# Fro116/RecommenderSystem

Hardware: AMD Instinct MI355X
Metric: interactions/sec (higher is better)
Workload: dtype bf16

## Files before the change

### include/rsys_debug.h

```cpp
#ifndef RSYS_DEBUG_H
#define RSYS_DEBUG_H
#include "rsys.h"

#ifdef __cplusplus
extern "C" {
#endif

int32_t rsys_debug_get(rsys_model* m, const char* key, void* out, int64_t bytes);

int32_t rsys_local_group_create(int32_t world, int32_t device, void** group);
int32_t rsys_local_group_destroy(void* group);
int32_t rsys_comm_init_local(void* group, int32_t rank, rsys_comm** out);
int32_t rsys_comm_debug_delay(rsys_comm* c, int32_t microseconds);

int32_t rsys_dev_alloc(void** p, size_t bytes);
int32_t rsys_dev_free(void* p);
int32_t rsys_dev_h2d(void* dst, const void* src, size_t bytes);
int32_t rsys_dev_d2h(void* dst, const void* src, size_t bytes);
int32_t rsys_dev_memset(void* dst, int value, size_t bytes);
int32_t rsys_op_gemm(int32_t dtype, const void* A, const void* B, void* C, int32_t M, int32_t N, int32_t K,
                     int64_t lda, int64_t ldb, int64_t ldc, int32_t a_km, int32_t b_km, int32_t a_f32, int32_t c_f32,
                     int32_t splitk);
int32_t rsys_op_gemm_rows(int32_t dtype, const void* A, const void* B, void* C, int32_t M, int32_t N, int32_t K,
                          int64_t lda, int64_t ldb, int64_t ldc, int32_t b_km, int32_t c_f32, const int32_t* rows_dev);
// ... 2 lines not shown
int32_t rsys_op_gemm_epi(int32_t dtype, const void* A, const void* B, void* C, int32_t M, int32_t N, int32_t K, int64_t lda,
                         int64_t ldb, int64_t ldc, int32_t b_km, int32_t c_f32, int32_t epi, float alpha, int32_t accum,
                         const float* bias, const float* resid, int64_t ldr, void* C2, int64_t ldc2, const float* E,
                         const float* rope_cos, const float* rope_sin, const float* rope_cs, const int32_t* rope_pos, int32_t T,
                         int32_t hd, int32_t n_q, int32_t n_k, const int32_t* m_dev, char* tag, int32_t tag_bytes, int32_t* half);
int32_t rsys_debug_gemm_route(int32_t dtype, int32_t M, int32_t N, int32_t K, int64_t lda, int64_t ldb, int64_t ldc, int32_t a_km,
                              int32_t b_km, int32_t a_f32, int32_t c_f32, int32_t epi, int32_t splitk, int32_t flags, float alpha,
                              int32_t accum, int32_t set, int32_t m_expect, int32_t cus, char* tag, int32_t tag_bytes, int32_t* splits);
int32_t rsys_op_attention(int32_t dtype, int32_t B, int32_t T, int32_t H, int32_t KV, int32_t hd, const void* qkv,
                          const int32_t* uid, const int32_t* tm, void* O, float* lse, const void* dO, void* dqkv,
                          const float* rope_cos, const float* rope_sin);
int32_t rsys_op_attention_ex(int32_t dtype, int32_t B, int32_t T, int32_t H, int32_t KV, int32_t hd, const void* qkv,
                             const int32_t* uid, const int32_t* tm, void* O, float* lse, const void* dO, void* dqkv,
                             const float* rope_cos, const float* rope_sin, const int32_t* rope_pos, int32_t rope_rows,
                             const int32_t* q_active, float* amax_fwd, float* amax_bwd);
int32_t rsys_op_attention_selected(int32_t dtype, int32_t B, int32_t T, int32_t H, int32_t KV, int32_t hd, const void* qkv,
                                   const int32_t* uid, const int32_t* tm, int32_t n_sel, const int32_t* sel, void* O);
int32_t rsys_op_attention_maps(int32_t dtype, int32_t B, int32_t T, int32_t H, int32_t KV, int32_t hd, const int32_t* uid, const int32_t* tm,
                               const int32_t* q_active, const int32_t* uid_prev, const int32_t* tm_prev, void* qmap, void* kmap,
                               void* qmap_full, void* kmap_full, void* qmap16, void* kmap16, uint64_t* qbits, uint64_t* kbits,
                               int32_t* order_q, int32_t* order_k, int32_t* info);
int32_t rsys_op_attention_cached(int32_t dtype, int32_t rows, int32_t T, int32_t H, int32_t KV, int32_t hd, const void* qkv, const void* cache,
                                 int32_t n_slots, const int32_t* slot, const int32_t* n_hist, const int32_t* n_cand, void* O);
int32_t rsys_op_attention_cached_tiles(int32_t dtype, int32_t rows, int32_t T, int32_t H, int32_t KV, int32_t hd, const void* qkv, const void* cache,
                                       int32_t n_slots, int32_t Tc, int32_t n_seg, const int32_t* seg, void* O);
int32_t rsys_op_rank_cache_copy_segments(int32_t dtype, int32_t rows, int32_t T, int32_t H, int32_t KV, int32_t hd, const void* qkv, void* cache,
                                         int32_t n_slots, int32_t Tc, int32_t n_seg, const int32_t* seg);
int32_t rsys_rank_cache_get(rsys_model* m, int32_t layer, int32_t slot, void* out, int64_t bytes);
int32_t rsys_op_topk(const float* scores, int64_t ld, int32_t rows, int32_t V, int32_t k,
                     int32_t* ids, float* vals, int32_t* counts);
int32_t rsys_op_topk_window(const float* scores, int64_t ld, int32_t rows, int32_t V, const int64_t* start, const int32_t* len,
                            int32_t* ids, float* vals, int32_t* counts, int32_t* totals, int32_t* bounds);
int32_t rsys_op_lse(const float* z, int64_t ldz, int32_t rows, int32_t V, float* lse);
int32_t rsys_op_text_rows(void* search, const float* x, int32_t n, float* z_out, float* lse_out);
int32_t rsys_op_query_weights(const float* z, int64_t ldz, const float* lse, const int32_t* members, const int32_t* ranges, int32_t q0,
                              const float* user_w, int32_t n_groups, const float* src, float* dst, int32_t V, int32_t last,
// ... 100 lines not shown
```

### recommendersystem_amd/_lib.py

```python
import ctypes as C
import os

os.environ.setdefault("HSA_ENABLE_IPC_MODE_LEGACY", "0")

HERE = os.path.dirname(os.path.abspath(__file__))
LIB_PATH = os.path.join(HERE, "librsys_hip.so")


class RsysError(RuntimeError):
    pass


class rsys_config(C.Structure):
    _fields_ = [
        ("num_layers", C.c_int32), ("num_heads", C.c_int32), ("num_kv_heads", C.c_int32),
        ("embed_dim", C.c_int32), ("intermediate_dim", C.c_int32), ("max_sequence_length", C.c_int32),
        ("vocab_0", C.c_int32), ("vocab_1", C.c_int32),
        ("vocab_status", C.c_int32), ("vocab_gender", C.c_int32), ("vocab_source", C.c_int32),
        ("metadata_dim", C.c_int32),
        ("min_ts", C.c_double), ("max_ts", C.c_double),
        ("rating_mean", C.c_float), ("rating_std", C.c_float), ("mask_rate", C.c_float),
        ("mask_topk", C.c_int32), ("finetune", C.c_int32), ("finetune_metric", C.c_int32),
        ("dtype", C.c_int32), ("max_rows", C.c_int32), ("lora_dropout", C.c_float),
        ("table_shard_rank", C.c_int32), ("table_shard_world", C.c_int32), ("sampled_negatives", C.c_int32),
# ... 127 lines not shown
    ("rsys_adapter_forward_backward", C.c_int32, [_P, C.c_int32, _P, _P, C.c_float, C.c_uint64, C.c_uint64]),
    ("rsys_adapter_forward_backward_packed", C.c_int32, [_P, C.c_int32, _P, C.c_int32, C.c_float, C.c_uint64, C.c_uint64]),
    ("rsys_adapter_grad_get", C.c_int32, [_P, C.c_int32, C.c_char_p, _P, C.c_int64]),
    ("rsys_adapter_zero_grad", C.c_int32, [_P]),
    ("rsys_adapter_adamw_step", C.c_int32, [_P, C.c_float, C.c_float, C.c_float, C.c_float, C.c_float, _P, C.c_int32, _P]),
    ("rsys_adapter_adamw_state_get", C.c_int32, [_P, C.c_int32, C.c_char_p, _P, _P, C.c_int64, C.POINTER(C.c_int32)]),
    ("rsys_adapter_adamw_state_set", C.c_int32, [_P, C.c_int32, C.c_char_p, _P, _P, C.c_int64, C.c_int32]),
    ("rsys_rank_cache_reserve", C.c_int32, [_P, C.c_int32]),
    ("rsys_rank_cache_store", C.c_int32, [_P, _P, _P, _P]),
    ("rsys_rank_cache_candidates", C.c_int32, [_P, _P, _P, _P, _P]),
    ("rsys_rank_cache_store_packed", C.c_int32, [_P, _P, C.c_int32, _P]),
    ("rsys_rank_cache_candidates_packed", C.c_int32, [_P, _P, C.c_int32, _P, _P]),
    ("rsys_rank_cache_get", C.c_int32, [_P, C.c_int32, C.c_int32, _P, C.c_int64]),
    ("rsys_op_attention_selected", C.c_int32, [C.c_int32] * 6 + [_P, _P, _P, C.c_int32, _P, _P]),
    ("rsys_op_attention_maps", C.c_int32, [C.c_int32] * 6 + [_P] * 16),
    ("rsys_op_attention_cached", C.c_int32, [C.c_int32] * 6 + [_P, _P, C.c_int32, _P, _P, _P, _P]),
    ("rsys_op_attention_cached_tiles", C.c_int32, [C.c_int32] * 6 + [_P, _P, C.c_int32, C.c_int32, C.c_int32, _P, _P]),
    ("rsys_op_rank_cache_copy_segments", C.c_int32, [C.c_int32] * 6 + [_P, _P, C.c_int32, C.c_int32, C.c_int32, _P]),
    ("rsys_trunk_output_get", C.c_int32, [_P, _P, C.c_int64]),
    ("rsys_debug_get", C.c_int32, [_P, C.c_char_p, _P, C.c_int64]),
    ("rsys_clip_grad_norm", C.c_int32, [_P, C.c_float, C.POINTER(C.c_float)]),
    ("rsys_adamw_create", C.c_int32, [_P, C.c_float, C.c_float, C.c_float, C.c_float, C.c_float, C.POINTER(_P)]),
    ("rsys_adamw_destroy", C.c_int32, [_P]),
    ("rsys_adamw_step", C.c_int32, [_P, C.c_float, C.c_float, C.c_float]),
    ("rsys_adamw_set_zero1", C.c_int32, [_P, C.c_int32, C.c_int32]),
    ("rsys_adamw_step_zero1", C.c_int32, [_P, _P, C.c_float, C.c_float, C.c_float]),
    ("rsys_adamw_state_get", C.c_int32, [_P, C.c_char_p, _P, _P, C.c_int64, C.POINTER(C.c_int32)]),
    ("rsys_adamw_state_set", C.c_int32, [_P, C.c_char_p, _P, _P, C.c_int64, C.c_int32]),
    ("rsys_comm_unique_id", C.c_int32, [C.POINTER(C.c_uint8 * 128)]),
    ("rsys_comm_init", C.c_int32, [C.POINTER(C.c_uint8 * 128), C.c_int32, C.c_int32, C.c_int32, C.POINTER(_P)]),
# ... 29 lines not shown
    ("rsys_op_gemm_f8", C.c_int32, [_P, _P, _P, C.c_int32, C.c_int32, C.c_int32, C.c_int64, C.c_int64, C.c_int64, C.c_int32, C.c_int32, _P,
                                      C.c_int32, C.c_int32, C.c_int32, C.c_int32, C.c_int32]),
    ("rsys_op_gemm_group", C.c_int32, [C.c_int32] + [_P] * 13 + [C.c_int32, C.c_int32, C.POINTER(C.c_int32), C.POINTER(C.c_int32)]),
    ("rsys_op_gemm_f8_splitk", C.c_int32, [_P, _P, _P, C.c_int32, C.c_int32, C.c_int32, C.c_int64, C.c_int64, C.c_int64, _P,
                                             C.c_int32, C.c_int32, C.c_int32]),
    ("rsys_op_gemm_rows", C.c_int32, [C.c_int32, _P, _P, _P, C.c_int32, C.c_int32, C.c_int32, C.c_int64, C.c_int64, C.c_int64,
                                      C.c_int32, C.c_int32, _P]),
    ("rsys_op_gemm_klimit", C.c_int32, [C.c_int32, _P, _P, _P, C.c_int32, C.c_int32, C.c_int32, C.c_int64, C.c_int64, C.c_int64, C.c_int32, _P]),
    ("rsys_op_gemm_epi", C.c_int32, [C.c_int32, _P, _P, _P, C.c_int32, C.c_int32, C.c_int32, C.c_int64, C.c_int64, C.c_int64, C.c_int32, C.c_int32,
                                     C.c_int32, C.c_float, C.c_int32, _P, _P, C.c_int64, _P, C.c_int64, _P, _P, _P, _P, _P,
                                     C.c_int32, C.c_int32, C.c_int32, C.c_int32, _P, C.c_char_p, C.c_int32, C.POINTER(C.c_int32)]),
    ("rsys_debug_gemm_route", C.c_int32, [C.c_int32] * 4 + [C.c_int64] * 3 + [C.c_int32] * 7 + [C.c_float] + [C.c_int32] * 4
                                          + [C.c_char_p, C.c_int32, C.POINTER(C.c_int32)]),
    ("rsys_op_attention", C.c_int32, [C.c_int32] + [C.c_int32] * 5 + [_P] * 9),
    ("rsys_op_attention_ex", C.c_int32, [C.c_int32] + [C.c_int32] * 5 + [_P] * 10 + [C.c_int32, _P, _P, _P]),
    ("rsys_op_query_weights", C.c_int32, [_P, C.c_int64, _P, _P, _P, C.c_int32, _P, C.c_int32, _P, _P, C.c_int32, C.c_int32,
                                          _P, _P, _P, _P, _P, _P, C.c_float, C.c_int32, _P,
                                          _P, _P, _P, C.c_int32, _P, _P, C.c_int32, _P, _P]),
    ("rsys_op_topk", C.c_int32, [_P, C.c_int64, C.c_int32, C.c_int32, C.c_int32, _P, _P, _P]),
    ("rsys_op_topk_window", C.c_int32, [_P, C.c_int64, C.c_int32, C.c_int32, _P, _P, _P, _P, _P, _P, _P]),
    ("rsys_op_lse", C.c_int32, [_P, C.c_int64, C.c_int32, C.c_int32, _P]),
    ("rsys_op_text_rows", C.c_int32, [_P, _P, C.c_int32, _P, _P]),
    ("rsys_op_target_rank", C.c_int32, [_P, C.c_int64, C.c_int32, C.c_int32, _P, _P]),
    ("rsys_op_pair_ranks", C.c_int32, [_P, C.c_int64, C.c_int32, C.c_int32, _P, _P, _P, _P]),
    ("rsys_rank_gram_get", C.c_int32, [_P, C.c_int32, C.c_int32, _P, _P, _P, C.c_int64]),
    ("rsys_op_rerank", C.c_int32, [C.c_int32, C.c_int32, _P, _P, _P, _P, _P, _P]),
    ("rsys_op_embedding_scatter", C.c_int32, [_P, C.c_int64, _P, _P, C.c_int32, C.c_int32, C.c_int32, _P, C.c_int32]),
    ("rsys_op_rmsnorm_fwd", C.c_int32, [C.c_int32, _P, _P, _P, _P, C.c_int64, C.c_int32, _P, _P, _P]),
    ("rsys_op_rmsnorm_bwd", C.c_int32, [C.c_int32, C.c_int32] + [_P] * 11 + [C.c_int64, C.c_int32, _P, C.c_int32]),
    ("rsys_op_ce", C.c_int32, [C.c_int32, _P, C.c_int64, C.c_int32, C.c_int32] + [_P] * 6 + [C.c_float, _P, C.c_int32]),
# ... 79 lines not shown
```

### recommendersystem_amd/csrc/attention.hip

```cpp
#include "attention_common.hpp"

namespace rsys {

template <typename T, int HD, bool DMA, int LG>
struct AttnKVStage {
  using W = typename AMap<LG>::W;
  static constexpr int TILE = DMA ? 64 * 64 : ACfg<T, HD>::TILE;
  const AttnParams& p;
  T* const Ks;
  T* const Vs;
  unsigned long long* const ab;
  const int t, l, w;
  W bits, fullbits, wbits;
  at_i32x4 k_rs, v_rs, qb_rs;
  TileOffs<T, HD> kv_of;
  bool w0;
  TileRegs<T, HD> rk, rv;
  unsigned long long rb = 0ull;
  int dv_[2] = {0, 0};

  __device__ __forceinline__ AttnKVStage(const AttnParams& p_, unsigned char* smem, int t_)
      : p(p_), Ks((T*)smem), Vs(Ks + 2 * TILE), ab((unsigned long long*)(Vs + 2 * TILE)), t(t_), l(t_ & 63), w(t_ >> 6) {}
  __device__ __forceinline__ void init(int b, int kvh, int qt) {
    const int nt = (p.T + 63) / 64;
// ... 326 lines not shown
    const T* krow = (const T*)p.k + (tok0 + kr) * p.ld + kvh * HD;
    const T* vrow = (const T*)p.v + (tok0 + kr) * p.ld + kvh * HD;
#pragma unroll
    for (int s = 0; s < 4; ++s) { kf[s] = *(const bf16x8*)(krow + 16 * s + 8 * h); vf[s] = *(const bf16x8*)(vrow + 16 * s + 8 * h); }
  }
  f32x16 dK[2], dV[2];
#pragma unroll
  for (int i = 0; i < 16; ++i) { dK[0][i] = 0.f; dK[1][i] = 0.f; dV[0][i] = 0.f; dV[1][i] = 0.f; }
  const int qa = p.q_active != nullptr ? p.q_active[b] : NTM;
  const W act = map_below<LG>(qa);
  const int t0i = b * nt + 2 * pr, t1i = min(2 * pr + 1, nt - 1) + b * nt;
  const W bits = map_uniform((W)((kmap[t0i] | (2 * pr + 1 < nt ? kmap[t1i] : (W)0)) & act));
  const int kti = b * nt + min(kvt, nt - 1);
  const W fullbits = tile_ok ? map_uniform(kmap_full[kti]) : (W)0;
  const W wbits = tile_ok ? map_uniform((W)(kmap16[kti * 4 + 2 * (w & 1)] | kmap16[kti * 4 + 2 * (w & 1) + 1])) : (W)0;
  const at_i32x4 q_rs = at_rsrc((const T*)p.q + tok0 * p.ld + kvh * rep * HD, ((long long)(p.T - 1) * p.ld + rep * HD) * sizeof(T));
  const at_i32x4 do_rs = at_rsrc((const T*)p.dO + tok0 * p.ldo + kvh * rep * HD, ((long long)(p.T - 1) * p.ldo + rep * HD) * sizeof(T));
  const at_i32x4 lse_rs = at_rsrc(p.lse + ((long long)b * p.H + kvh * rep) * p.T, (long long)rep * p.T * 4);
  const at_i32x4 dl_rs = at_rsrc(p.delta + ((long long)b * p.H + kvh * rep) * p.T, (long long)rep * p.T * 4);
  const at_i32x4 kb_rs = at_rsrc(p.kbits + (long long)kti * nt * 64, tile_ok ? (long long)nt * 64 * 8 : 0);
  int qv_[2], dv_[2];
#pragma unroll
  for (int k = 0; k < 2; ++k) {
    const int row = 16 * w + 8 * k + (l >> 3), ch = (l & 7) ^ sw32(row);
    qv_[k] = (int)((row * p.ld + ch * 8) * sizeof(T));
    dv_[k] = (int)((row * p.ldo + ch * 8) * sizeof(T));
  }
  const int G = h ^ sw32(r32);
  const int i16 = l & 15, g16 = (l >> 4) & 1;
  const int Lc = (2 * g16 + ((i16 & 3) >> 1)) ^ ((((i16 >> 2) >> 1) & 1) << 2 | (h << 1));
// ... 34 lines not shown
  for (int s = 0; s < 4; ++s) asm volatile("" : "+v"(kf[s]), "+v"(vf[s]));
  asm volatile("" : "+v"(wk));
  __syncthreads();
  tr_[1] = KVT_NOW();
  while (it < end) {
    [[maybe_unused]] const unsigned long long ta = KVT_NOW();
    const int nxt = next_item(it + 1);
    if (nxt < end) stage(nxt, cur ^ 1);
    [[maybe_unused]] const unsigned long long tb = KVT_NOW();
    if ((wbits >> (it & (NTM - 1))) & 1u) {
      const bool fullt = (fullbits >> (it & (NTM - 1))) & 1u;
      const unsigned char* Qc = Qb + cur * (TB * 2);
      const unsigned char* dOc = dOb + cur * (TB * 2);
#pragma unroll
      for (int qb = 0; qb < 2; ++qb) {
        f32x16 S, dP;
#pragma unroll
        for (int k = 0; k < 4; ++k) {
          const float4 l4 = *(const float4*)(lse2 + cur * 64 + 32 * qb + 8 * k + 4 * h);
          const float4 d4 = *(const float4*)(dls + cur * 64 + 32 * qb + 8 * k + 4 * h);
          S[4 * k] = l4.x; S[4 * k + 1] = l4.y; S[4 * k + 2] = l4.z; S[4 * k + 3] = l4.w;
          dP[4 * k] = d4.x; dP[4 * k + 1] = d4.y; dP[4 * k + 2] = d4.z; dP[4 * k + 3] = d4.w;
        }
#pragma unroll
        for (int s = 0; s < 4; ++s) {
          S = mfma32(*(const bf16x8*)(Qc + qb * 4096 + a_row[s]), kf[s], S);
          dP = mfma32(*(const bf16x8*)(dOc + qb * 4096 + a_row[s]), vf[s], dP);
        }
        const unsigned int w32 = (unsigned int)(qb ? (wk >> 32) : wk);
        if (!fullt && __builtin_amdgcn_ballot_w64(w32 != 0xFFFFFFFFu) != 0ull) {
// ... 255 lines not shown
  if (rc) return rc;
  if constexpr (is_bf16<T>::value && HD == 64) {
    if (attn_kv_pairs(p)) {
      const int npair = ((p.T + 63) / 64 + 1) / 2;
      hipLaunchKernelGGL(attn_bwd_kv32_kernel<LG>, dim3(npair * p.KV * p.B), dim3(256), 4 * 64 * 64 * 2 + 256 * 4, s, p);
      HIP_CHECK(hipGetLastError());
      return RSYS_OK;
    }
  }
  hipLaunchKernelGGL((attn_bwd_kv_kernel<T, HD, LG>), dim3(((p.T + 63) / 64) * p.KV * p.B), dim3(256), sm_kv, s, p);
  HIP_CHECK(hipGetLastError());
  return RSYS_OK;
}

template <typename T>
int launch_attn_bwd(const AttnParams& p, hipStream_t s) {
  int rc = check_attn(p, sizeof(T));
  if (rc) return rc;
  ARG_CHECK(p.H / p.KV <= 8, "attention: at most 8 query heads per kv head");
  return attn_for_hd_lg(p, [&](auto hd, auto lg) { return attn_bwd_hd<T, decltype(hd)::value, decltype(lg)::value>(p, s); });
}
template int launch_attn_bwd<bf16>(const AttnParams&, hipStream_t);
template int launch_attn_bwd<float>(const AttnParams&, hipStream_t);

}

#ifdef ATTN_KV_TRACE
extern "C" __attribute__((visibility("default"))) int rsys_attn_trace_read(void* dst, unsigned long long n) {
  return (int)hipMemcpyFromSymbol(dst, HIP_SYMBOL(rsys::rsys_attn_trace), n);
}
#endif
// ... 1 lines not shown
```

### recommendersystem_amd/csrc/attention_maps.hip

```cpp
#include "attention_common.hpp"

namespace rsys {

#define KEY_NO_Q ((int)0xFFFFE000u)
#define KEY_NO_K ((int)0xFFFFFFFFu)
__device__ __forceinline__ int token_key(int uid, int tm) { return (int)(((unsigned int)uid << 12) | (unsigned int)tm); }

extern "C" __device__ int rsys_at_writelane(int value, int lane, int old) __asm("llvm.amdgcn.writelane.i32");
template <int LG>
__global__ __launch_bounds__(256) void attn_tilemap_kernel(AttnParams p) {
  using W = typename AMap<LG>::W;
  constexpr int NTM = 1 << LG;
  __shared__ W any_bits, any16[4];
  __shared__ unsigned int kany[NTM];
  __shared__ int cnt[NTM];
  __shared__ unsigned short kcols[NTM][64][4];
  __shared__ int keys[64 * NTM];
  __shared__ int qkeys[64];
  const int qt = blockIdx.x, b = blockIdx.y, t = threadIdx.x, l = t & 63, w = t >> 6;
  const int nt = (p.T + 63) / 64;
  const long long base = (long long)b * p.T;
  if (t == 0) any_bits = 0u;
  if (t < 4) any16[t] = 0u;
  if (t < NTM) { cnt[t] = 0; kany[t] = 0u; }
  for (int i = t; i < nt * 64; i += 256) keys[i] = i < p.T ? token_key(p.uid[base + i], p.tm[base + i]) : KEY_NO_K;
  int myq = KEY_NO_Q;
  if (l < 16) { const int q = qt * 64 + w * 16 + l; if (q < p.T) myq = token_key(p.uid[base + q], p.tm[base + q]); }
  if (l < 16) qkeys[w * 16 + l] = myq;
  __syncthreads();
  int aq[16], aq0[16];
// ... 14 lines not shown
    }
    if (n) {
      int qlo = 0, qhi = 0;
#pragma unroll
      for (int i = 0; i < 16; ++i) {
        const bool hit = ak == aq[i] || ak == aq0[i];
        const unsigned long long hb = __ballot(hit);
        qlo = rsys_at_writelane((int)(unsigned int)hb, i, qlo);
        qhi = rsys_at_writelane((int)(unsigned int)(hb >> 32), i, qhi);
        kcol |= hit ? (1u << i) : 0u;
      }
      qrow = ((unsigned long long)(unsigned int)qhi << 32) | (unsigned int)qlo;
    }
    if (l < 16) p.qbits[(((long long)b * nt + qt) * nt + j) * 64 + w * 16 + l] = qrow;
    kcols[j][l][w] = (unsigned short)kcol;
    if (n) {
      wany |= (W)1 << j;
      const unsigned long long km = __ballot(mine);
      unsigned int kg = 0u;
#pragma unroll
      for (int g4 = 0; g4 < 4; ++g4) kg |= ((km >> (16 * g4)) & 0xFFFFull) ? (1u << g4) : 0u;
      if (l == 0) { atomicAdd(&cnt[j], n); atomicOr(&kany[j], kg); }
    }
  }
  if (l == 0) { any16[w] = wany; atomicOr(&any_bits, wany); }
  __syncthreads();
  for (int c = t; c < nt * 64; c += 256)
    p.kbits[(((long long)b * nt + (c >> 6)) * nt + qt) * 64 + (c & 63)] = *(const unsigned long long*)kcols[c >> 6][c & 63];
  if (t < nt) {
    const bool any = (any_bits >> t) & 1u, full = cnt[t] == 4096;
    if (any) atomicOr(&map_ptr<LG>(p.kmap)[b * nt + t], (W)1 << qt);
    if (full) atomicOr(&map_ptr<LG>(p.kmap_full)[b * nt + t], (W)1 << qt);
    if (full) atomicOr(&map_ptr<LG>(p.qmap_full)[b * nt + qt], (W)1 << t);
    const unsigned int kg = kany[t];
#pragma unroll
    for (int g4 = 0; g4 < 4; ++g4)
      if ((kg >> g4) & 1u) atomicOr(&map_ptr<LG>(p.kmap16)[(b * nt + t) * 4 + g4], (W)1 << qt);
  }
  if (t == 0) map_ptr<LG>(p.qmap)[b * nt + qt] = any_bits;
  if (t < 4) map_ptr<LG>(p.qmap16)[(b * nt + qt) * 4 + t] = any16[t];
}

static int attn_order_chunk_cap(int lg) { return lg == 5 ? 400 : 200; }
template <int LG>
__global__ __launch_bounds__(256) void attn_order_kernel(AttnParams p, int R, int identity, int kv_pairs) {
  using W = typename AMap<LG>::W;
  constexpr int NTM = 1 << LG, OS = NTM + 2;
  const W *qmap = map_ptr<LG>(p.qmap), *kmap = map_ptr<LG>(p.kmap);
  extern __shared__ int ocnt[];
  const int side = blockIdx.y, nt = (p.T + 63) / 64, n_groups = p.B * p.KV;
  const int n_inner = side == 0 ? (p.H / p.KV / R) * nt : (kv_pairs ? (nt + 1) / 2 : nt);
  int* out = side == 0 ? p.order_q : p.order_k;
// ... 49 lines not shown
  }
}

AttnOrderPlan attn_order_plan(const AttnParams& p) {
  AttnOrderPlan o{};
  const int nt = (p.T + 63) / 64, n_groups = p.B * p.KV;
  o.R = attn_heads_per_wg(p); o.kv_pairs = attn_kv_pairs(p) ? 1 : 0;
  o.lists = (n_groups & 7) == 0 ? 8 : 1;
  o.n_inner_q = (p.H / p.KV / o.R) * nt; o.n_inner_k = o.kv_pairs ? (nt + 1) / 2 : nt;
  const int ns_max = (n_groups / o.lists) * (p.H / p.KV) * nt;
  o.chunk_cap = attn_order_chunk_cap(nt > 32 ? 6 : 5); o.chunks = (ns_max + 63) / 64;
  o.identity = o.chunks > o.chunk_cap ? 1 : 0;
  return o;
}

int launch_attn_tilemap(const AttnParams& p, hipStream_t s) {
  ARG_CHECK(p.T % 8 == 0 && (p.T + 63) / 64 <= 64, "attention: T must be a multiple of 8 and <= 4096");
  ARG_CHECK(p.qbits != nullptr && p.kbits != nullptr, "attention: the pair-bit buffers (AttnParams::qbits / kbits) are required");
  const bool wide = (p.T + 63) / 64 > 32;
  ARG_CHECK(p.maps_zero_base != nullptr, "attention: the tile maps come from attn_maps_alloc (AttnParams::maps_zero_base)");
  HIP_CHECK(hipMemsetAsync(p.maps_zero_base, 0, p.maps_zero_bytes, s));
  if (wide) hipLaunchKernelGGL(attn_tilemap_kernel<6>, dim3((p.T + 63) / 64, p.B), dim3(256), 0, s, p);
  else hipLaunchKernelGGL(attn_tilemap_kernel<5>, dim3((p.T + 63) / 64, p.B), dim3(256), 0, s, p);
  if (p.order_q != nullptr || p.order_k != nullptr) {
    const AttnOrderPlan o = attn_order_plan(p);
    const dim3 og(o.lists, 2);
    const size_t rows = (size_t)(std::min(o.chunks, o.chunk_cap) + 1);
    if (wide) hipLaunchKernelGGL(attn_order_kernel<6>, og, dim3(256), rows * 66 * 4, s, p, o.R, o.identity, o.kv_pairs);
    else hipLaunchKernelGGL(attn_order_kernel<5>, og, dim3(256), rows * 34 * 4, s, p, o.R, o.identity, o.kv_pairs);
  }
  HIP_CHECK(hipGetLastError());
// ... 5 lines not shown
```

### recommendersystem_amd/csrc/capi_ops.hip

```cpp
#include <algorithm>
#include <string.h>

#include "model_internal.hpp"

using namespace rsys;

namespace {
struct HookScratch {
  const char* who;
  std::vector<void*> bufs;
  explicit HookScratch(const char* who_) : who(who_) {}
  ~HookScratch() { hipDeviceSynchronize(); for (void* p : bufs) hipFree(p); }
  int alloc(void** p, size_t bytes) {
    if (hipMalloc(p, bytes ? bytes : 16) != hipSuccess) {
      (void)hipGetLastError();
      *p = nullptr;
      set_error(std::string(who) + ": no device memory for the call's scratch");
      return RSYS_ERR_HIP;
    }
    bufs.push_back(*p);
    return RSYS_OK;
  }
  template <typename T> int get(T** p, size_t count) { return alloc((void**)p, count * sizeof(T)); }
};
// ... 34 lines not shown
    set_error(std::string(who) + ": the ordered (deterministic) branch did not run");
    return RSYS_ERR_STATE;
  }
};
int hook_ints(const int32_t* dev, long long n, std::vector<int>& out) {
  out.resize((size_t)std::max(n, 0LL));
  if (n > 0) HIP_CHECK(hipMemcpy(out.data(), dev, (size_t)n * 4, hipMemcpyDeviceToHost));
  return RSYS_OK;
}
int hook_attn_maps(HookScratch& scratch, AttnParams& p, AttnMaps& maps, bool fill = false, const int32_t* uid_prev = nullptr,
                   const int32_t* tm_prev = nullptr) {
  RC(attn_maps_alloc(maps, p.B, p.T, p.H, p.KV, [&](void** b, size_t bytes) { return scratch.alloc(b, bytes); }));
  maps.apply(p);
  if (fill) {
    const size_t nt = (size_t)(p.T + 63) / 64;
    HIP_CHECK(hipMemsetAsync(maps.zero_base, 0xA5, 12 * maps.map_bytes, nullptr));
    HIP_CHECK(hipMemsetAsync(maps.order_q, 0xA5, (size_t)p.B * p.H * nt * 4, nullptr));
    HIP_CHECK(hipMemsetAsync(maps.order_k, 0xA5, (size_t)p.B * p.KV * nt * 4, nullptr));
    HIP_CHECK(hipMemsetAsync(maps.qbits, 0xA5, (size_t)p.B * nt * nt * 64 * 8, nullptr));
    HIP_CHECK(hipMemsetAsync(maps.kbits, 0xA5, (size_t)p.B * nt * nt * 64 * 8, nullptr));
  }
  if (uid_prev != nullptr) {
    AttnParams prev = p;
    prev.uid = uid_prev; prev.tm = tm_prev;
    RC(launch_attn_tilemap(prev, nullptr));
  }
  return launch_attn_tilemap(p, nullptr);
}
GemmParams hook_dw_params(const void* A, const void* B, void* C, int32_t M, int32_t N, int32_t K, int64_t lda, int64_t ldb, int64_t ldc,
                          int32_t f8, const float* f8_desc, int32_t f8_rseg, int32_t f8_rowmode) {
  GemmParams p{};
// ... 171 lines not shown
  switches_parse();
  ARG_CHECK(A8 != nullptr && B8 != nullptr && C != nullptr, "rsys_op_gemm_f8_splitk: null operand");
  ARG_CHECK(launches >= 1, "rsys_op_gemm_f8_splitk: launches >= 1");
  const GemmParams p = hook_dw_params(A8, B8, C, M, N, K, lda, ldb, ldc, 2, desc_dev, rseg, rowmode);
  int rc = RSYS_OK;
  for (int i = 0; i < launches && rc == RSYS_OK; ++i) rc = launch_gemm8p_f8_splitk(p, nullptr);
  return hook_finish(rc);
}

int32_t rsys_op_attention(int32_t dtype, int32_t B, int32_t T, int32_t H, int32_t KV, int32_t hd, const void* qkv,
                          const int32_t* uid, const int32_t* tm, void* O, float* lse, const void* dO, void* dqkv,
                          const float* rope_cos, const float* rope_sin) {
  return rsys_op_attention_ex(dtype, B, T, H, KV, hd, qkv, uid, tm, O, lse, dO, dqkv, rope_cos, rope_sin, nullptr, T, nullptr, nullptr, nullptr);
}

int32_t rsys_op_attention_ex(int32_t dtype, int32_t B, int32_t T, int32_t H, int32_t KV, int32_t hd, const void* qkv,
                             const int32_t* uid, const int32_t* tm, void* O, float* lse, const void* dO, void* dqkv,
                             const float* rope_cos, const float* rope_sin, const int32_t* rope_pos, int32_t rope_rows,
                             const int32_t* q_active, float* amax_fwd, float* amax_bwd) {
  switches_parse();
  ARG_CHECK(dtype == RSYS_DTYPE_BF16 || dtype == RSYS_DTYPE_FP32, "rsys_op_attention: dtype fp32 or bf16");
  ARG_CHECK(B >= 1 && T >= 1 && H >= 1 && KV >= 1 && qkv && uid && tm && O && lse, "rsys_op_attention: null or empty");
  ARG_CHECK(!dO || (dqkv && rope_cos && rope_sin), "rsys_op_attention: the backward needs dqkv and the rope tables");
  if (dO && rope_pos) {
    std::vector<int32_t> pos((size_t)B * T);
    HIP_CHECK(hipMemcpy(pos.data(), rope_pos, pos.size() * 4, hipMemcpyDeviceToHost));
    for (int32_t v : pos) ARG_CHECK(v >= 0 && v < rope_rows, "rsys_op_attention: rope_pos outside the tables");
  } else if (dO) {
    ARG_CHECK(rope_rows >= T, "rsys_op_attention: rope tables shorter than T");
  }
  const size_t e = dtype == RSYS_DTYPE_BF16 ? 2 : 4;
  AttnParams p{};
  p.B = B; p.T = T; p.H = H; p.KV = KV; p.hd = hd; p.is_bf16 = dtype == RSYS_DTYPE_BF16;
  p.q = qkv; p.k = (const unsigned char*)qkv + (size_t)H * hd * e; p.v = (const unsigned char*)qkv + (size_t)(H + KV) * hd * e;
  p.ld = (long long)(H + 2 * KV) * hd;
  p.o = O; p.ldo = (long long)H * hd; p.lse = lse; p.uid = uid; p.tm = tm;
  HookScratch scratch("rsys_op_attention");
  AttnMaps maps; float* delta = nullptr;
  RC(scratch.get(&delta, (size_t)B * H * T));
  p.delta = delta;
  p.dO = dO; p.dq = dqkv; p.dk = (unsigned char*)dqkv + (size_t)H * hd * e;
  p.dv = (unsigned char*)dqkv + (size_t)(H + KV) * hd * e; p.ldg = p.ld;
  p.rope_cos = rope_cos; p.rope_sin = rope_sin; p.rope_pos = rope_pos; p.q_active = q_active;
  if (q_active) HIP_CHECK(hipMemsetAsync(delta, 0xFF, sizeof(float) * B * H * T, nullptr));
  int rc = hook_attn_maps(scratch, p, maps);
  p.f8_amax = amax_fwd;
  if (!rc) rc = BY_DTYPE(dtype, launch_attn_fwd<Elt>(p, nullptr));
  p.f8_amax = amax_bwd;
  if (!rc && dO) rc = BY_DTYPE(dtype, launch_attn_bwd<Elt>(p, nullptr));
  return hook_finish(rc);
}

int32_t rsys_op_attention_selected(int32_t dtype, int32_t B, int32_t T, int32_t H, int32_t KV, int32_t hd, const void* qkv, const int32_t* uid,
                                   const int32_t* tm, int32_t n_sel, const int32_t* sel, void* O) {
  switches_parse();
  ARG_CHECK(dtype == RSYS_DTYPE_BF16 || dtype == RSYS_DTYPE_FP32, "rsys_op_attention_selected: dtype fp32 or bf16");
  ARG_CHECK(B >= 1 && T >= 1 && H >= 1 && KV >= 1 && n_sel >= 1 && qkv && uid && tm && sel && O, "rsys_op_attention_selected: null or empty");
  ARG_CHECK((long long)B * T < (1ll << 31), "rsys_op_attention_selected: B * T must stay below 2^31");
  {
    std::vector<int32_t> hs((size_t)n_sel);
    HIP_CHECK(hipMemcpy(hs.data(), sel, hs.size() * 4, hipMemcpyDeviceToHost));
    for (int32_t v : hs) ARG_CHECK(v >= 0 && v < B * T, "rsys_op_attention_selected: a selected token outside [0, B * T)");
  }
  const size_t e = dtype == RSYS_DTYPE_BF16 ? 2 : 4;
  AttnParams p{};
// ... 45 lines not shown
  RC(hook_finish(hook_attn_maps(scratch, p, maps, true, uid_prev, tm_prev)));
  const size_t mapb = (size_t)B * nt * 4 * attn_map_words(T), bitb = (size_t)B * nt * nt * 64 * 8;
  HIP_CHECK(hipMemcpy(qmap, maps.qmap, mapb, hipMemcpyDeviceToHost));
  HIP_CHECK(hipMemcpy(kmap, maps.kmap, mapb, hipMemcpyDeviceToHost));
  HIP_CHECK(hipMemcpy(qmap_full, maps.qmap_full, mapb, hipMemcpyDeviceToHost));
  HIP_CHECK(hipMemcpy(kmap_full, maps.kmap_full, mapb, hipMemcpyDeviceToHost));
  HIP_CHECK(hipMemcpy(qmap16, maps.qmap16, 4 * mapb, hipMemcpyDeviceToHost));
  HIP_CHECK(hipMemcpy(kmap16, maps.kmap16, 4 * mapb, hipMemcpyDeviceToHost));
  HIP_CHECK(hipMemcpy(qbits, maps.qbits, bitb, hipMemcpyDeviceToHost));
  HIP_CHECK(hipMemcpy(kbits, maps.kbits, bitb, hipMemcpyDeviceToHost));
  HIP_CHECK(hipMemcpy(order_q, maps.order_q, (size_t)B * H * nt * 4, hipMemcpyDeviceToHost));
  HIP_CHECK(hipMemcpy(order_k, maps.order_k, (size_t)B * KV * nt * 4, hipMemcpyDeviceToHost));
  const AttnOrderPlan o = attn_order_plan(p);
  const int32_t facts[8] = {attn_map_words(T), o.R, o.kv_pairs, o.lists == 8 ? 1 : 0, o.n_inner_q, o.n_inner_k, o.identity, (int32_t)nt};
  memcpy(info, facts, sizeof(facts));
  return RSYS_OK;
}

int32_t rsys_op_attention_cached(int32_t dtype, int32_t rows, int32_t T, int32_t H, int32_t KV, int32_t hd, const void* qkv, const void* cache,
                                 int32_t n_slots, const int32_t* slot, const int32_t* n_hist, const int32_t* n_cand, void* O) {
  switches_parse();
  ARG_CHECK(dtype == RSYS_DTYPE_BF16 || dtype == RSYS_DTYPE_FP32, "dtype: fp32 or bf16");
  ARG_CHECK(qkv && cache && slot && n_hist && n_cand && O && KV >= 1 && H >= 1, "null or empty");
  CandAttnParams p{};
  p.rows = rows; p.T = T; p.H = H; p.KV = KV; p.hd = hd;
  p.qkv = qkv; p.ld = (long long)(H + 2 * KV) * hd; p.cache = cache; p.n_slots = n_slots;
  p.slot = slot; p.n_hist = n_hist; p.n_cand = n_cand; p.o = O; p.ldo = (long long)H * hd;
  return hook_finish(BY_DTYPE(dtype, launch_attn_cand<Elt>(p, nullptr)));
}

// ... 561 lines not shown
```

### recommendersystem_amd/csrc/kernels.hpp

```cpp
#pragma once
#include "common.hpp"

namespace rsys {

static inline int div_up(long long a, long long b) { return (int)((a + b - 1) / b); }

struct BatchDev {
  int N, rows, S;
  const int *userid, *tmid, *gender, *source, *matchedid, *status;
  const double* time;
  const float *rating, *progress;
  const float* label[6]; const float* weight[6]; const int* position[6];
  const unsigned char *watch_mask, *rating_mask;
  const int* rope_pos;
  int *m_tmid, *m_matchedid, *m_status;
  float *m_rating, *m_progress;
  float* m_label[4]; float* m_weight[4]; int* m_position[4];
};

struct DetScratch {
  float* part = nullptr; long long cap = 0; float* tmp = nullptr; long long tmp_cap = 0;
  int part_used = 0, part_short = 0;
};
extern thread_local DetScratch g_det;
// ... 124 lines not shown

int launch_action_small_bwd(const float* gf , const BatchDev& b, const SmallParams& sp,
                            float* g_per_cos, float* g_per_sin, float* g_status, float* g_gender, float* g_source,
                            hipStream_t s);

struct AttnParams {
  int B, T, H, KV, hd;
  int is_bf16;
  const void *q, *k, *v;
  long long ld;
  void* o; long long ldo;
  float* lse;
  const int *uid, *tm;
  unsigned int *qmap, *kmap, *qmap_full, *kmap_full;
  unsigned int *qmap16, *kmap16;
  const int* q_active;
  void* maps_zero_base; size_t maps_zero_bytes;
  const void* dO; float* delta;
  void *dq, *dk, *dv; long long ldg;
  const float *rope_cos, *rope_sin; const int* rope_pos;
  float* f8_amax;
  int *order_q, *order_k;
  unsigned long long *qbits, *kbits;
};
inline int attn_map_words(int T) { return (T + 63) / 64 > 32 ? 2 : 1; }
struct AttnMaps {
  unsigned int *qmap = nullptr, *kmap = nullptr, *qmap_full = nullptr, *kmap_full = nullptr, *qmap16 = nullptr, *kmap16 = nullptr;
  int *order_q = nullptr, *order_k = nullptr;
  unsigned long long *qbits = nullptr, *kbits = nullptr;
  void* zero_base = nullptr; size_t zero_bytes = 0;
  size_t map_bytes = 0;
  void apply(AttnParams& p) const {
    p.qmap = qmap; p.kmap = kmap; p.qmap_full = qmap_full; p.kmap_full = kmap_full; p.qmap16 = qmap16; p.kmap16 = kmap16;
    p.order_q = order_q; p.order_k = order_k; p.qbits = qbits; p.kbits = kbits;
    p.maps_zero_base = zero_base; p.maps_zero_bytes = zero_bytes;
  }
};
template <typename Alloc>
int attn_maps_alloc(AttnMaps& a, long long rows, int T, int H, int KV, Alloc&& alloc) {
  const long long nt = (T + 63) / 64;
  const long long mb = (rows * nt * 4 * attn_map_words(T) + 255) / 256 * 256;
  unsigned char* base = nullptr;
  if (int rc = alloc((void**)&base, (size_t)(mb * 12))) return rc;
  a.kmap = (unsigned int*)base; a.kmap_full = (unsigned int*)(base + mb); a.qmap_full = (unsigned int*)(base + 2 * mb); a.kmap16 = (unsigned int*)(base + 3 * mb);
  a.qmap = (unsigned int*)(base + 7 * mb); a.qmap16 = (unsigned int*)(base + 8 * mb);
  a.zero_base = base; a.zero_bytes = (size_t)(7 * mb); a.map_bytes = (size_t)mb;
  if (int rc = alloc((void**)&a.order_q, (size_t)(rows * H * nt * 4))) return rc;
  if (int rc = alloc((void**)&a.order_k, (size_t)(rows * KV * nt * 4))) return rc;
  if (int rc = alloc((void**)&a.qbits, (size_t)(rows * nt * nt * 64 * 8))) return rc;
  return alloc((void**)&a.kbits, (size_t)(rows * nt * nt * 64 * 8));
}
struct AttnOrderPlan { int R, kv_pairs, lists, n_inner_q, n_inner_k, identity, chunk_cap, chunks; };
AttnOrderPlan attn_order_plan(const AttnParams& p);
int launch_attn_tilemap(const AttnParams& p, hipStream_t s);
struct CandAttnParams {
  int rows, T, H, KV, hd;
  const void* qkv; long long ld;
  const void* cache; int n_slots;
  int Tc;
  const int *slot, *n_hist, *n_cand;
  void* o; long long ldo;
// ... 60 lines not shown
```

### recommendersystem_amd/csrc/switches.hip

```cpp
#include "switches.hpp"

#include <cstdio>
#include <cstdlib>
#include <cstring>
#include <mutex>

namespace rsys {
namespace {

struct Entry { const char* name; int Switches::*field; int dflt; };
const Entry kEntries[] = {
    {"RSYS_ATTN_DMA", &Switches::attn_dma, 1},
    {"RSYS_GEMM_KERNEL", &Switches::gemm_kernel, -1},
    {"RSYS_GEMM_KERNEL_TN", &Switches::gemm_kernel_tn, -1},
    {"RSYS_GEMM_KERNEL_NT_SPLITK", &Switches::gemm_kernel_nt_splitk, -1},
    {"RSYS_GEMM_KERNEL_MIX", &Switches::gemm_kernel_mix, 1},
    {"RSYS_GEMM8C_HALF", &Switches::gemm8c_half, 1},
    {"RSYS_GEMM4P", &Switches::gemm4p, 1},
    {"RSYS_GEMM4K", &Switches::gemm4k, 1},
    {"RSYS_GEMM8C", &Switches::gemm8c, 1},
    {"RSYS_GEMM_REVERSE", &Switches::gemm_reverse, 1},
    {"RSYS_GEMM_PATCH", &Switches::gemm_patch, 1},
    {"RSYS_TABLE_TAIL", &Switches::table_tail, 1},
    {"RSYS_DW_GROUP", &Switches::dw_group, 1},
    {"RSYS_DET_DW_GROUP", &Switches::det_dw_group, 1},
    {"RSYS_SPARSE_TOP", &Switches::sparse_top, 1},
    {"RSYS_TOP_ORDER", &Switches::top_order, 1},
// ... 53 lines not shown
```

### recommendersystem_amd/csrc/switches.hpp

```cpp
#pragma once

namespace rsys {

struct Switches {
  int attn_dma;
  int gemm_kernel;
  int gemm_kernel_tn;
  int gemm_kernel_nt_splitk;
  int gemm_kernel_mix;
  int gemm8c_half;
  int gemm4p;
  int gemm4k;
  int gemm8c;
  int gemm_reverse;
  int gemm_patch;
  int table_tail;
  int dw_group;
  int det_dw_group;
  int sparse_top;
  int top_order;
  int select_chunked;
  int scatter_atomic;
  int f8_dw;
  int f8_dw_round_bf16;
// ... 18 lines not shown
```

Baseline: 1.631 million.

## Skip fully masked 32x32 sub-blocks in attention backward via block-none maps

The tile-map kernel now also records, per key tile and query tile, which 32x32 quadrants contain no allowed pairs, and stores them in a new kblk_none map region. The attention backward kernel loads these bits and skips the S/dP MFMA work for empty sub-blocks inside partially masked tiles. This targets wasted compute on sparse user/time masks. It costs a larger map allocation, extra atomics in the map kernel, and a per-iteration branch. A switch can disable it, and debug entry points expose delta and the block maps.

```diff
diff --git a/include/rsys_debug.h b/include/rsys_debug.h
--- a/include/rsys_debug.h
+++ b/include/rsys_debug.h
@@ -40,12 +40,18 @@
                              const int32_t* uid, const int32_t* tm, void* O, float* lse, const void* dO, void* dqkv,
                              const float* rope_cos, const float* rope_sin, const int32_t* rope_pos, int32_t rope_rows,
                              const int32_t* q_active, float* amax_fwd, float* amax_bwd);
+int32_t rsys_op_attention_delta(int32_t dtype, int32_t B, int32_t T, int32_t H, int32_t KV, int32_t hd, const void* qkv,
+                                const int32_t* uid, const int32_t* tm, void* O, float* lse, const void* dO, void* dqkv,
+                                const float* rope_cos, const float* rope_sin, const int32_t* rope_pos, int32_t rope_rows,
+                                const int32_t* q_active, float* delta);
 int32_t rsys_op_attention_selected(int32_t dtype, int32_t B, int32_t T, int32_t H, int32_t KV, int32_t hd, const void* qkv,
                                    const int32_t* uid, const int32_t* tm, int32_t n_sel, const int32_t* sel, void* O);
 int32_t rsys_op_attention_maps(int32_t dtype, int32_t B, int32_t T, int32_t H, int32_t KV, int32_t hd, const int32_t* uid, const int32_t* tm,
                                const int32_t* q_active, const int32_t* uid_prev, const int32_t* tm_prev, void* qmap, void* kmap,
                                void* qmap_full, void* kmap_full, void* qmap16, void* kmap16, uint64_t* qbits, uint64_t* kbits,
                                int32_t* order_q, int32_t* order_k, int32_t* info);
+int32_t rsys_op_attention_block_maps(int32_t dtype, int32_t B, int32_t T, int32_t H, int32_t KV, int32_t hd, const int32_t* uid,
+                                     const int32_t* tm, void* kblk_none);
 int32_t rsys_op_attention_cached(int32_t dtype, int32_t rows, int32_t T, int32_t H, int32_t KV, int32_t hd, const void* qkv, const void* cache,
                                  int32_t n_slots, const int32_t* slot, const int32_t* n_hist, const int32_t* n_cand, void* O);
 int32_t rsys_op_attention_cached_tiles(int32_t dtype, int32_t rows, int32_t T, int32_t H, int32_t KV, int32_t hd, const void* qkv, const void* cache,
diff --git a/recommendersystem_amd/_lib.py b/recommendersystem_amd/_lib.py
--- a/recommendersystem_amd/_lib.py
+++ b/recommendersystem_amd/_lib.py
@@ -165,6 +165,7 @@
     ("rsys_rank_cache_get", C.c_int32, [_P, C.c_int32, C.c_int32, _P, C.c_int64]),
     ("rsys_op_attention_selected", C.c_int32, [C.c_int32] * 6 + [_P, _P, _P, C.c_int32, _P, _P]),
     ("rsys_op_attention_maps", C.c_int32, [C.c_int32] * 6 + [_P] * 16),
+    ("rsys_op_attention_block_maps", C.c_int32, [C.c_int32] * 6 + [_P] * 3),
     ("rsys_op_attention_cached", C.c_int32, [C.c_int32] * 6 + [_P, _P, C.c_int32, _P, _P, _P, _P]),
     ("rsys_op_attention_cached_tiles", C.c_int32, [C.c_int32] * 6 + [_P, _P, C.c_int32, C.c_int32, C.c_int32, _P, _P]),
     ("rsys_op_rank_cache_copy_segments", C.c_int32, [C.c_int32] * 6 + [_P, _P, C.c_int32, C.c_int32, C.c_int32, _P]),
@@ -224,6 +225,7 @@
                                           + [C.c_char_p, C.c_int32, C.POINTER(C.c_int32)]),
     ("rsys_op_attention", C.c_int32, [C.c_int32] + [C.c_int32] * 5 + [_P] * 9),
     ("rsys_op_attention_ex", C.c_int32, [C.c_int32] + [C.c_int32] * 5 + [_P] * 10 + [C.c_int32, _P, _P, _P]),
+    ("rsys_op_attention_delta", C.c_int32, [C.c_int32] + [C.c_int32] * 5 + [_P] * 10 + [C.c_int32, _P, _P]),
     ("rsys_op_query_weights", C.c_int32, [_P, C.c_int64, _P, _P, _P, C.c_int32, _P, C.c_int32, _P, _P, C.c_int32, C.c_int32,
                                           _P, _P, _P, _P, _P, _P, C.c_float, C.c_int32, _P,
                                           _P, _P, _P, C.c_int32, _P, _P, C.c_int32, _P, _P]),
diff --git a/recommendersystem_amd/csrc/attention.hip b/recommendersystem_amd/csrc/attention.hip
--- a/recommendersystem_amd/csrc/attention.hip
+++ b/recommendersystem_amd/csrc/attention.hip
@@ -364,6 +364,11 @@
   const int kti = b * nt + min(kvt, nt - 1);
   const W fullbits = tile_ok ? map_uniform(kmap_full[kti]) : (W)0;
   const W wbits = tile_ok ? map_uniform((W)(kmap16[kti * 4 + 2 * (w & 1)] | kmap16[kti * 4 + 2 * (w & 1) + 1])) : (W)0;
+  W bnone[2] = {(W)0, (W)0};
+  if (p.kblk_none != nullptr && tile_ok) {
+#pragma unroll
+    for (int qb = 0; qb < 2; ++qb) bnone[qb] = map_uniform(map_ptr<LG>(p.kblk_none)[kti * 4 + 2 * (w & 1) + qb]);
+  }
   const at_i32x4 q_rs = at_rsrc((const T*)p.q + tok0 * p.ld + kvh * rep * HD, ((long long)(p.T - 1) * p.ld + rep * HD) * sizeof(T));
   const at_i32x4 do_rs = at_rsrc((const T*)p.dO + tok0 * p.ldo + kvh * rep * HD, ((long long)(p.T - 1) * p.ldo + rep * HD) * sizeof(T));
   const at_i32x4 lse_rs = at_rsrc(p.lse + ((long long)b * p.H + kvh * rep) * p.T, (long long)rep * p.T * 4);
@@ -428,6 +433,7 @@
       const unsigned char* dOc = dOb + cur * (TB * 2);
 #pragma unroll
       for (int qb = 0; qb < 2; ++qb) {
+        if ((bnone[qb] >> (it & (NTM - 1))) & 1u) continue;
         f32x16 S, dP;
 #pragma unroll
         for (int k = 0; k < 4; ++k) {
@@ -713,7 +719,9 @@
 }
 
 template <typename T>
-int launch_attn_bwd(const AttnParams& p, hipStream_t s) {
+int launch_attn_bwd(const AttnParams& p0, hipStream_t s) {
+  AttnParams p = p0;
+  if (sw().attn_blocks == 0) p.kblk_none = nullptr;
   int rc = check_attn(p, sizeof(T));
   if (rc) return rc;
   ARG_CHECK(p.H / p.KV <= 8, "attention: at most 8 query heads per kv head");
diff --git a/recommendersystem_amd/csrc/attention_maps.hip b/recommendersystem_amd/csrc/attention_maps.hip
--- a/recommendersystem_amd/csrc/attention_maps.hip
+++ b/recommendersystem_amd/csrc/attention_maps.hip
@@ -14,6 +14,7 @@
   __shared__ W any_bits, any16[4];
   __shared__ unsigned int kany[NTM];
   __shared__ int cnt[NTM];
+  __shared__ unsigned char wkg[NTM][4];
   __shared__ unsigned short kcols[NTM][64][4];
   __shared__ int keys[64 * NTM];
   __shared__ int qkeys[64];
@@ -58,14 +59,15 @@
     }
     if (l < 16) p.qbits[(((long long)b * nt + qt) * nt + j) * 64 + w * 16 + l] = qrow;
     kcols[j][l][w] = (unsigned short)kcol;
+    unsigned int kg = 0u;
     if (n) {
       wany |= (W)1 << j;
       const unsigned long long km = __ballot(mine);
-      unsigned int kg = 0u;
 #pragma unroll
       for (int g4 = 0; g4 < 4; ++g4) kg |= ((km >> (16 * g4)) & 0xFFFFull) ? (1u << g4) : 0u;
       if (l == 0) { atomicAdd(&cnt[j], n); atomicOr(&kany[j], kg); }
     }
+    if (l == 0) wkg[j][w] = (unsigned char)kg;
   }
   if (l == 0) { any16[w] = wany; atomicOr(&any_bits, wany); }
   __syncthreads();
@@ -80,6 +82,15 @@
 #pragma unroll
     for (int g4 = 0; g4 < 4; ++g4)
       if ((kg >> g4) & 1u) atomicOr(&map_ptr<LG>(p.kmap16)[(b * nt + t) * 4 + g4], (W)1 << qt);
+  }
+  if (p.kblk_none != nullptr && t < nt) {
+#pragma unroll
+    for (int qh = 0; qh < 2; ++qh) {
+      const unsigned int g2 = (unsigned int)wkg[t][2 * qh] | (unsigned int)wkg[t][2 * qh + 1];
+#pragma unroll
+      for (int kh = 0; kh < 2; ++kh)
+        if (((g2 >> (2 * kh)) & 3u) == 0u) atomicOr(&map_ptr<LG>(p.kblk_none)[(b * nt + t) * 4 + 2 * kh + qh], (W)1 << qt);
+    }
   }
   if (t == 0) map_ptr<LG>(p.qmap)[b * nt + qt] = any_bits;
   if (t < 4) map_ptr<LG>(p.qmap16)[(b * nt + qt) * 4 + t] = any16[t];
@@ -159,7 +170,9 @@
   return o;
 }
 
-int launch_attn_tilemap(const AttnParams& p, hipStream_t s) {
+int launch_attn_tilemap(const AttnParams& p0, hipStream_t s) {
+  AttnParams p = p0;
+  if (sw().attn_blocks == 0) p.kblk_none = nullptr;
   ARG_CHECK(p.T % 8 == 0 && (p.T + 63) / 64 <= 64, "attention: T must be a multiple of 8 and <= 4096");
   ARG_CHECK(p.qbits != nullptr && p.kbits != nullptr, "attention: the pair-bit buffers (AttnParams::qbits / kbits) are required");
   const bool wide = (p.T + 63) / 64 > 32;
diff --git a/recommendersystem_amd/csrc/capi_ops.hip b/recommendersystem_amd/csrc/capi_ops.hip
--- a/recommendersystem_amd/csrc/capi_ops.hip
+++ b/recommendersystem_amd/csrc/capi_ops.hip
@@ -72,7 +72,7 @@
   maps.apply(p);
   if (fill) {
     const size_t nt = (size_t)(p.T + 63) / 64;
-    HIP_CHECK(hipMemsetAsync(maps.zero_base, 0xA5, 12 * maps.map_bytes, nullptr));
+    HIP_CHECK(hipMemsetAsync(maps.zero_base, 0xA5, ATTN_MAP_BLOCKS * maps.map_bytes, nullptr));
     HIP_CHECK(hipMemsetAsync(maps.order_q, 0xA5, (size_t)p.B * p.H * nt * 4, nullptr));
     HIP_CHECK(hipMemsetAsync(maps.order_k, 0xA5, (size_t)p.B * p.KV * nt * 4, nullptr));
     HIP_CHECK(hipMemsetAsync(maps.qbits, 0xA5, (size_t)p.B * nt * nt * 64 * 8, nullptr));
@@ -274,10 +274,10 @@
   return rsys_op_attention_ex(dtype, B, T, H, KV, hd, qkv, uid, tm, O, lse, dO, dqkv, rope_cos, rope_sin, nullptr, T, nullptr, nullptr, nullptr);
 }
 
-int32_t rsys_op_attention_ex(int32_t dtype, int32_t B, int32_t T, int32_t H, int32_t KV, int32_t hd, const void* qkv,
-                             const int32_t* uid, const int32_t* tm, void* O, float* lse, const void* dO, void* dqkv,
-                             const float* rope_cos, const float* rope_sin, const int32_t* rope_pos, int32_t rope_rows,
-                             const int32_t* q_active, float* amax_fwd, float* amax_bwd) {
+static int32_t op_attention(int32_t dtype, int32_t B, int32_t T, int32_t H, int32_t KV, int32_t hd, const void* qkv,
+                            const int32_t* uid, const int32_t* tm, void* O, float* lse, const void* dO, void* dqkv,
+                            const float* rope_cos, const float* rope_sin, const int32_t* rope_pos, int32_t rope_rows,
+                            const int32_t* q_active, float* amax_fwd, float* amax_bwd, float* delta_out) {
   switches_parse();
   ARG_CHECK(dtype == RSYS_DTYPE_BF16 || dtype == RSYS_DTYPE_FP32, "rsys_op_attention: dtype fp32 or bf16");
   ARG_CHECK(B >= 1 && T >= 1 && H >= 1 && KV >= 1 && qkv && uid && tm && O && lse, "rsys_op_attention: null or empty");
@@ -296,8 +296,8 @@
   p.ld = (long long)(H + 2 * KV) * hd;
   p.o = O; p.ldo = (long long)H * hd; p.lse = lse; p.uid = uid; p.tm = tm;
   HookScratch scratch("rsys_op_attention");
-  AttnMaps maps; float* delta = nullptr;
-  RC(scratch.get(&delta, (size_t)B * H * T));
+  AttnMaps maps; float* delta = delta_out;
+  if (delta == nullptr) RC(scratch.get(&delta, (size_t)B * H * T));
   p.delta = delta;
   p.dO = dO; p.dq = dqkv; p.dk = (unsigned char*)dqkv + (size_t)H * hd * e;
   p.dv = (unsigned char*)dqkv + (size_t)(H + KV) * hd * e; p.ldg = p.ld;
@@ -309,6 +309,20 @@
   p.f8_amax = amax_bwd;
   if (!rc && dO) rc = BY_DTYPE(dtype, launch_attn_bwd<Elt>(p, nullptr));
   return hook_finish(rc);
+}
+
+int32_t rsys_op_attention_ex(int32_t dtype, int32_t B, int32_t T, int32_t H, int32_t KV, int32_t hd, const void* qkv,
+                             const int32_t* uid, const int32_t* tm, void* O, float* lse, const void* dO, void* dqkv,
+                             const float* rope_cos, const float* rope_sin, const int32_t* rope_pos, int32_t rope_rows,
+                             const int32_t* q_active, float* amax_fwd, float* amax_bwd) {
+  return op_attention(dtype, B, T, H, KV, hd, qkv, uid, tm, O, lse, dO, dqkv, rope_cos, rope_sin, rope_pos, rope_rows, q_active, amax_fwd, amax_bwd, nullptr);
+}
+int32_t rsys_op_attention_delta(int32_t dtype, int32_t B, int32_t T, int32_t H, int32_t KV, int32_t hd, const void* qkv,
+                                const int32_t* uid, const int32_t* tm, void* O, float* lse, const void* dO, void* dqkv,
+                                const float* rope_cos, const float* rope_sin, const int32_t* rope_pos, int32_t rope_rows,
+                                const int32_t* q_active, float* delta) {
+  ARG_CHECK(dO && delta, "rsys_op_attention_delta: the backward's operands and the delta buffer are required");
+  return op_attention(dtype, B, T, H, KV, hd, qkv, uid, tm, O, lse, dO, dqkv, rope_cos, rope_sin, rope_pos, rope_rows, q_active, nullptr, nullptr, delta);
 }
 
 int32_t rsys_op_attention_selected(int32_t dtype, int32_t B, int32_t T, int32_t H, int32_t KV, int32_t hd, const void* qkv, const int32_t* uid,
@@ -384,6 +398,33 @@
   const AttnOrderPlan o = attn_order_plan(p);
   const int32_t facts[8] = {attn_map_words(T), o.R, o.kv_pairs, o.lists == 8 ? 1 : 0, o.n_inner_q, o.n_inner_k, o.identity, (int32_t)nt};
   memcpy(info, facts, sizeof(facts));
+  return RSYS_OK;
+}
+
+int32_t rsys_op_attention_block_maps(int32_t dtype, int32_t B, int32_t T, int32_t H, int32_t KV, int32_t hd, const int32_t* uid,
+                                     const int32_t* tm, void* kblk_none) {
+  switches_parse();
+  ARG_CHECK(dtype == RSYS_DTYPE_BF16 || dtype == RSYS_DTYPE_FP32, "rsys_op_attention_block_maps: dtype fp32 or bf16");
+  ARG_CHECK(B >= 1 && T >= 1 && H >= 1 && KV >= 1 && hd >= 1 && uid && tm, "rsys_op_attention_block_maps: null or empty");
+  ARG_CHECK(H % KV == 0, "rsys_op_attention_block_maps: H must be a multiple of KV");
+  ARG_CHECK(T % 8 == 0 && T <= 4096, "rsys_op_attention_block_maps: T must be a multiple of 8 and <= 4096");
+  ARG_CHECK(kblk_none, "rsys_op_attention_block_maps: null output");
+  const size_t nt = (size_t)(T + 63) / 64, n_tok = (size_t)B * T;
+  {
+    std::vector<int> h;
+    RC(hook_ints(uid, (long long)n_tok, h));
+    for (int v : h) ARG_CHECK(v >= 0 && v < (1 << 19), "rsys_op_attention_block_maps: a uid outside [0, 2^19)");
+    RC(hook_ints(tm, (long long)n_tok, h));
+    for (int v : h) ARG_CHECK(v >= 0 && v < 4096, "rsys_op_attention_block_maps: a tm outside [0, 4096)");
+  }
+  AttnParams p{};
+  p.B = B; p.T = T; p.H = H; p.KV = KV; p.hd = hd; p.is_bf16 = dtype == RSYS_DTYPE_BF16;
+  p.uid = uid; p.tm = tm;
+  HookScratch scratch("rsys_op_attention_block_maps");
+  AttnMaps maps;
+  RC(hook_finish(hook_attn_maps(scratch, p, maps, true)));
+  const size_t mapb = (size_t)B * nt * 4 * attn_map_words(T);
+  HIP_CHECK(hipMemcpy(kblk_none, maps.kblk_none, 4 * mapb, hipMemcpyDeviceToHost));
   return RSYS_OK;
 }
 
diff --git a/recommendersystem_amd/csrc/kernels.hpp b/recommendersystem_amd/csrc/kernels.hpp
--- a/recommendersystem_amd/csrc/kernels.hpp
+++ b/recommendersystem_amd/csrc/kernels.hpp
@@ -162,6 +162,7 @@
   const int *uid, *tm;
   unsigned int *qmap, *kmap, *qmap_full, *kmap_full;
   unsigned int *qmap16, *kmap16;
+  unsigned int* kblk_none;
   const int* q_active;
   void* maps_zero_base; size_t maps_zero_bytes;
   const void* dO; float* delta;
@@ -174,25 +175,29 @@
 inline int attn_map_words(int T) { return (T + 63) / 64 > 32 ? 2 : 1; }
 struct AttnMaps {
   unsigned int *qmap = nullptr, *kmap = nullptr, *qmap_full = nullptr, *kmap_full = nullptr, *qmap16 = nullptr, *kmap16 = nullptr;
+  unsigned int* kblk_none = nullptr;
   int *order_q = nullptr, *order_k = nullptr;
   unsigned long long *qbits = nullptr, *kbits = nullptr;
   void* zero_base = nullptr; size_t zero_bytes = 0;
   size_t map_bytes = 0;
   void apply(AttnParams& p) const {
     p.qmap = qmap; p.kmap = kmap; p.qmap_full = qmap_full; p.kmap_full = kmap_full; p.qmap16 = qmap16; p.kmap16 = kmap16;
+    p.kblk_none = kblk_none;
     p.order_q = order_q; p.order_k = order_k; p.qbits = qbits; p.kbits = kbits;
     p.maps_zero_base = zero_base; p.maps_zero_bytes = zero_bytes;
   }
 };
+constexpr int ATTN_MAP_BLOCKS = 16;
 template <typename Alloc>
 int attn_maps_alloc(AttnMaps& a, long long rows, int T, int H, int KV, Alloc&& alloc) {
   const long long nt = (T + 63) / 64;
   const long long mb = (rows * nt * 4 * attn_map_words(T) + 255) / 256 * 256;
   unsigned char* base = nullptr;
-  if (int rc = alloc((void**)&base, (size_t)(mb * 12))) return rc;
+  if (int rc = alloc((void**)&base, (size_t)(mb * ATTN_MAP_BLOCKS))) return rc;
   a.kmap = (unsigned int*)base; a.kmap_full = (unsigned int*)(base + mb); a.qmap_full = (unsigned int*)(base + 2 * mb); a.kmap16 = (unsigned int*)(base + 3 * mb);
-  a.qmap = (unsigned int*)(base + 7 * mb); a.qmap16 = (unsigned int*)(base + 8 * mb);
-  a.zero_base = base; a.zero_bytes = (size_t)(7 * mb); a.map_bytes = (size_t)mb;
+  a.kblk_none = (unsigned int*)(base + 7 * mb);
+  a.qmap = (unsigned int*)(base + 11 * mb); a.qmap16 = (unsigned int*)(base + 12 * mb);
+  a.zero_base = base; a.zero_bytes = (size_t)(11 * mb); a.map_bytes = (size_t)mb;
   if (int rc = alloc((void**)&a.order_q, (size_t)(rows * H * nt * 4))) return rc;
   if (int rc = alloc((void**)&a.order_k, (size_t)(rows * KV * nt * 4))) return rc;
   if (int rc = alloc((void**)&a.qbits, (size_t)(rows * nt * nt * 64 * 8))) return rc;
diff --git a/recommendersystem_amd/csrc/switches.hip b/recommendersystem_amd/csrc/switches.hip
--- a/recommendersystem_amd/csrc/switches.hip
+++ b/recommendersystem_amd/csrc/switches.hip
@@ -11,6 +11,7 @@
 struct Entry { const char* name; int Switches::*field; int dflt; };
 const Entry kEntries[] = {
     {"RSYS_ATTN_DMA", &Switches::attn_dma, 1},
+    {"RSYS_ATTN_BLOCKS", &Switches::attn_blocks, 1},
     {"RSYS_GEMM_KERNEL", &Switches::gemm_kernel, -1},
     {"RSYS_GEMM_KERNEL_TN", &Switches::gemm_kernel_tn, -1},
     {"RSYS_GEMM_KERNEL_NT_SPLITK", &Switches::gemm_kernel_nt_splitk, -1},
diff --git a/recommendersystem_amd/csrc/switches.hpp b/recommendersystem_amd/csrc/switches.hpp
--- a/recommendersystem_amd/csrc/switches.hpp
+++ b/recommendersystem_amd/csrc/switches.hpp
@@ -4,6 +4,7 @@
 
 struct Switches {
   int attn_dma;
+  int attn_blocks;
   int gemm_kernel;
   int gemm_kernel_tn;
   int gemm_kernel_nt_splitk;
```

After: 1.629 million. No clear change (-0.1%).
